# glmanhtu/vit-ed

Hardware: AMD Instinct MI355X
Metric: patch-pairs/sec fwd+bwd, div2k_erosion7_4bin_patch8_64 ViT-ED (higher is better)
Workload: dtype bf16

## Files before the change

### profiles/row_probe.py

```python
#!/usr/bin/env python3
import argparse
import os
import sys

import torch

sys.path.insert(0, os.path.dirname(os.path.dirname(os.path.abspath(__file__))))
import vited_amd as v

ops, L = v.ops, v._lib


def main():
    ap = argparse.ArgumentParser()
    ap.add_argument('--reps', type=int, default=10)
    ap.add_argument('--rows', type=int, nargs='*', default=[65536, 66560])
    a = ap.parse_args()
    dev = torch.device('cuda:0')
    g = torch.Generator(device='cpu').manual_seed(0)

    def rnd(*shape, scale=1.0):
        return (torch.randn(*shape, generator=g) * scale).to(dev)

    def timed(fn):
        for _ in range(3):
            fn()
        torch.cuda.synchronize()
        e0, e1 = torch.cuda.Event(enable_timing=True), torch.cuda.Event(enable_timing=True)
        e0.record()
        for _ in range(a.reps):
            fn()
        e1.record()
        torch.cuda.synchronize()
        return e0.elapsed_time(e1) / a.reps * 1e3

    N = 384
    print(f'{"shape":28s} {"two kernels":>12s} {"fused":>9s}   GB/s (fused, algorithmic)')
    for M in a.rows:
        gamma, beta, bias = 1.0 + rnd(N, scale=0.1), rnd(N, scale=0.1), rnd(N, scale=0.1)
        res = rnd(M, N)
        mean, rstd = rnd(M, scale=0.1), 1.0 + rnd(M, scale=0.1).abs()
        for K in (384, 768, 1152, 1536):
            x_lp, w = rnd(M, K).bfloat16(), rnd(N, K, scale=K ** -0.5).bfloat16()

            def fwd_two():
                y = ops.gemm(x_lp, w, epilogue=L.EPI_RESIDUAL, bias=bias, residual=res)
                return ops.layernorm_fwd(y, gamma, beta, 1e-6, torch.bfloat16)

            def fwd_fused():
                return ops.linear_residual_layernorm_fwd(x_lp, w, bias, res, gamma, beta, 1e-6)

            def bwd_two():
                dh = ops.gemm(x_lp, w)
                return ops.layernorm_bwd(dh, res, gamma, mean, rstd, dx_in=res, want_lp=True)

            def bwd_fused():
                return ops.linear_layernorm_bwd(x_lp, w, res, gamma, mean, rstd, dx_in=res, want_lp=True)

            t2, t1 = timed(fwd_two), timed(fwd_fused)
            byt = M * K * 2 + N * K * 2 + M * N * (4 + 4 + 2)
            print(f'fwd M={M} K={K:5d}          {t2:10.1f}us {t1:8.1f}us   {byt / t1 / 1e3:7.0f}   {2.0 * M * N * K / t1 / 1e6:6.0f} TF/s')
            t2, t1 = timed(bwd_two), timed(bwd_fused)
            byt = M * K * 2 + N * K * 2 + M * N * (4 + 4 + 4 + 2)
            print(f'bwd M={M} K={K:5d}          {t2:10.1f}us {t1:8.1f}us   {byt / t1 / 1e3:7.0f}   {2.0 * M * N * K / t1 / 1e6:6.0f} TF/s')


if __name__ == '__main__':
    main()
```

### vit-ed_amd/csrc/gemm_row.hip

```cpp
#include <mutex>
#include <type_traits>

#include "gemm_kernels.h"
#include "gemm_lds.h"

#define ROW_N 384
#define ROW_LD 388

enum { ROW_MODE_FWD = 0, ROW_MODE_BWD = 1 };

struct RowArgs {
    const bf16* A; int64_t lda;
    int seg_k; int64_t seg_stride;
    const bf16* W; int64_t ldw;
    int64_t M; int K;
    const float* bias; const float* residual; int64_t ldr;
    float* y; int64_t ldy;
    const float* gamma; const float* beta; float eps;
    bf16* h; int64_t ldh; float* mean; float* rstd;
    const float* x; int64_t ldx; const float* mean_in; const float* rstd_in;
    const float* dx_in; int64_t ldxi; float* dx; int64_t lddx; bf16* dx_lp; int64_t ldlp;
    float* partial;
};

template <int MT> struct RowCfg {
    static_assert(MT == 6 || MT == 8 || MT == 9 || MT == 10, "tile heights: 96, 128, 144 or 160 rows");
    static constexpr int BM = 16 * MT;
    static constexpr int A_BYTES = BM * 128;
    static constexpr int W_BYTES = ROW_N * 128;
    static constexpr int W_BASE = 3 * A_BYTES;
    static constexpr int LDS_BYTES = 3 * A_BYTES + 2 * W_BYTES;
    static constexpr int P0 = (MT + 1) / 2;
    static constexpr int A_PIECES = 2 * MT;
    static constexpr int A_J = (A_PIECES + 3) / 4;
    static constexpr int PASS_SUB = MT == 8 ? 4 : MT == 10 ? 5 : 3;
    static constexpr int PASS_ROWS = 16 * PASS_SUB;
    static constexpr int NPASS = MT / PASS_SUB;
    static constexpr int ROWS_PER_HALF = PASS_ROWS / 16;
    static constexpr bool EPI_ALL_ROWS = MT <= 9;
    static_assert(MT % PASS_SUB == 0, "passes cover the tile");
    static_assert(LDS_BYTES <= 160 * 1024, "LDS");
    static_assert(LDS_BYTES >= PASS_ROWS * ROW_LD * 4, "epilogue scratch must fit the staging buffers");
    static_assert(LDS_BYTES >= 16 * 2 * ROW_N * 4, "column-partial combine must fit the staging buffers");
};

__device__ __forceinline__ float row_half_sum(float v) { return half_wave_sum(v); }

#define ROW_STORE(ptr, val) __builtin_nontemporal_store(val, ptr)
#define ROW_STORE_LP(ptr, val) (*(ptr) = (val))
#define ROW_LOAD(ptr) __builtin_nontemporal_load(ptr)

struct RowFwdIn { f32x4 res[3]; };
struct RowBwdIn { f32x4 x[3], din[3]; float mu, rs; };

template <int MODE, int MT>
__global__ void __launch_bounds__(512)
gemm_row_kernel(const RowArgs a) {
    extern __shared__ __attribute__((aligned(16))) char smem[];
    using R = RowCfg<MT>;
    const int lane = threadIdx.x & 63;
    const int wave = __builtin_amdgcn_readfirstlane(threadIdx.x >> 6);
    const int64_t m0 = (int64_t)blockIdx.x * R::BM;

    f32x4 acc[MT][3];
#pragma unroll
    for (int i = 0; i < MT; ++i)
#pragma unroll
        for (int j = 0; j < 3; ++j) acc[i][j] = f32x4{0.f, 0.f, 0.f, 0.f};

    const int grp = wave >> 2, u = wave & 3;
    const int nt = a.K / 64;
    const int r8 = lane >> 3, c8 = lane & 7;
    const int cs_even = (c8 ^ (r8 >> 1)) * 8, cs_odd = (c8 ^ (r8 >> 1) ^ 4) * 8;
    const int cs_u = (u & 1) ? cs_odd : cs_even;
    const int a_per = (R::A_PIECES - u + 3) / 4;
    const bf16* pa[R::A_J];
#pragma unroll
    for (int j = 0; j < R::A_J; ++j) {
        int64_t ar = m0 + 8 * (4 * j + u) + r8;
#ifdef ROW_DBG_A_RESIDENT
        ar -= m0;
#endif
        ar = ar < a.M ? ar : a.M - 1;
        pa[j] = a.A + ar * a.lda + cs_u;
    }
    const bf16* pw = a.W + (int64_t)(8 * u + r8) * a.ldw + cs_u;
    auto issue_a = [&](int t) {
#ifdef ROW_DBG_NO_DMA
        return;
#endif
        if (t >= nt) return;
        char* dst = smem + (t % 3) * R::A_BYTES;
        const int k0 = t * 64;
        const int seg = k0 / a.seg_k;
        const int64_t ka = (int64_t)seg * a.seg_stride + (k0 - seg * a.seg_k);
#pragma unroll
        for (int j = 0; j < R::A_J; ++j)
            if (4 * j + 3 < R::A_PIECES || j < a_per) glds16_asm(pa[j] + ka, dst + (4 * j + u) * 1024);
    };
    auto issue_w = [&](int t, int part) {
#ifdef ROW_DBG_NO_DMA
        return;
#endif
        if (t >= nt) return;
        char* dst = smem + R::W_BASE + (t & 1) * R::W_BYTES + (16 * part + u) * 1024;
        const int64_t off = (int64_t)(128 * part) * a.ldw + t * 64;
#pragma unroll
        for (int j = 0; j < 4; ++j) glds16_asm(pw + off + (int64_t)(32 * j) * a.ldw, dst + 4 * j * 1024);
    };
    const int fr = lane & 15, fq = lane >> 4;
    const int loff0 = fr * 128 + ((fq ^ ((fr >> 1) & 7)) << 4), loff1 = fr * 128 + (((4 + fq) ^ ((fr >> 1) & 7)) << 4);
    bf16x8 fa[R::P0][2] = {}, fb[3][2] = {};
    auto read_b = [&](int t) {
#ifdef ROW_DBG_NO_READS
        return;
#endif
        const char* wb = smem + R::W_BASE + (t & 1) * R::W_BYTES + wave * 48 * 128;
#pragma unroll
        for (int j = 0; j < 3; ++j) {
            fb[j][0] = *(const bf16x8*)(wb + j * 2048 + loff0);
            fb[j][1] = *(const bf16x8*)(wb + j * 2048 + loff1);
        }
    };
    auto read_a = [&](int t, auto i0_tag, auto n_tag) {
        constexpr int I0 = decltype(i0_tag)::value, NR = decltype(n_tag)::value;
#ifdef ROW_DBG_NO_READS
        return;
#endif
        const char* ab = smem + (t % 3) * R::A_BYTES + I0 * 2048;
#pragma unroll
        for (int i = 0; i < NR; ++i) {
            fa[i][0] = *(const bf16x8*)(ab + i * 2048 + loff0);
            fa[i][1] = *(const bf16x8*)(ab + i * 2048 + loff1);
        }
    };
    auto mfmas = [&](auto i0_tag, auto n_tag) {
        constexpr int I0 = decltype(i0_tag)::value, NR = decltype(n_tag)::value;
        __builtin_amdgcn_s_setprio(1);
#pragma unroll
        for (int kk = 0; kk < 2; ++kk)
#pragma unroll
            for (int i = 0; i < NR; ++i)
#pragma unroll
                for (int j = 0; j < 3; ++j)
#ifdef ROW_DBG_NO_MFMA
                    asm volatile("" ::"v"(fb[j][kk]), "v"(fa[i][kk]));
#else
                    acc[I0 + i][j] = __builtin_amdgcn_mfma_f32_16x16x32_bf16(fb[j][kk], fa[i][kk], acc[I0 + i][j], 0, 0, 0);
#endif
        __builtin_amdgcn_s_setprio(0);
    };
    auto barrier = [&]() {
        __builtin_amdgcn_s_barrier();
        asm volatile("" ::: "memory");
    };
    auto certify_barrier = [&](bool younger) {
        __builtin_amdgcn_sched_barrier(0);
        if (!younger) asm volatile("s_waitcnt vmcnt(0)\n\ts_barrier" ::: "memory");
        else if (grp == 0 && a_per == 5) asm volatile("s_waitcnt vmcnt(5)\n\ts_barrier" ::: "memory");
        else if (grp == 0 && a_per == 3) asm volatile("s_waitcnt vmcnt(3)\n\ts_barrier" ::: "memory");
        else asm volatile("s_waitcnt vmcnt(4)\n\ts_barrier" ::: "memory");
        __builtin_amdgcn_sched_barrier(0);
    };
    auto landed = [&]() {
#ifndef ROW_DBG_LATE_LGKM
        __builtin_amdgcn_s_waitcnt(0xc07f);
#endif
    };
    using I0 = std::integral_constant<int, 0>;
    using IP0 = std::integral_constant<int, R::P0>;
    using IP1 = std::integral_constant<int, MT - R::P0>;
    if (grp == 0) {
        issue_a(0);
        issue_w(0, 1);
        issue_a(1);
        certify_barrier(nt > 1);
        for (int t = 0; t < nt; ++t) {
            read_b(t);
            read_a(t, I0{}, IP0{});
            issue_w(t + 1, 1);
            landed();
            barrier();
            mfmas(I0{}, IP0{});
            barrier();
            read_a(t, IP0{}, IP1{});
            issue_a(t + 2);
            landed();
            barrier();
            mfmas(IP0{}, IP1{});
            certify_barrier(t + 2 < nt);
        }
        barrier();
    } else {
        issue_w(0, 0);
        issue_w(0, 2);
        issue_w(1, 0);
        certify_barrier(nt > 1);
        barrier();
        for (int t = 0; t < nt; ++t) {
            read_b(t);
            read_a(t, I0{}, IP0{});
            issue_w(t + 1, 2);
            landed();
            barrier();
            mfmas(I0{}, IP0{});
            barrier();
            read_a(t, IP0{}, IP1{});
            issue_w(t + 2, 0);
            landed();
            certify_barrier(t + 2 < nt);
            mfmas(IP0{}, IP1{});
            barrier();
        }
    }
#ifdef ROW_DBG_NO_EPI
#pragma unroll
    for (int i = 0; i < MT; ++i)
#pragma unroll
        for (int j = 0; j < 3; ++j) asm volatile("" ::"v"(acc[i][j]));
    return;
#endif

    float* sc = (float*)smem;
    const int hl = lane & 31;
    const int hw = wave * 2 + (lane >> 5);
    const float inv_d = 1.0f / ROW_N;
    f32x4 gm[3], bt[3], bs[3];
#pragma unroll
    for (int j = 0; j < 3; ++j) {
        const int c = (j * 32 + hl) * 4;
        gm[j] = a.gamma ? *(const f32x4*)(a.gamma + c) : f32x4{1.f, 1.f, 1.f, 1.f};
        bt[j] = (MODE == ROW_MODE_FWD && a.beta) ? *(const f32x4*)(a.beta + c) : f32x4{0.f, 0.f, 0.f, 0.f};
        bs[j] = (MODE == ROW_MODE_FWD && a.bias) ? *(const f32x4*)(a.bias + c) : f32x4{0.f, 0.f, 0.f, 0.f};
    }
    f32x4 dg[3], db[3];
#pragma unroll
    for (int j = 0; j < 3; ++j) {
        dg[j] = f32x4{0.f, 0.f, 0.f, 0.f};
        db[j] = f32x4{0.f, 0.f, 0.f, 0.f};
    }
    auto load_fwd = [&](RowFwdIn& in, int64_t m) {
        const bool ok = m < a.M;
#pragma unroll
        for (int j = 0; j < 3; ++j)
            in.res[j] = ok ? ROW_LOAD((const f32x4*)(a.residual + m * a.ldr + (j * 32 + hl) * 4)) : f32x4{0.f, 0.f, 0.f, 0.f};
    };
    auto load_bwd = [&](RowBwdIn& in, int64_t m) {
        const bool ok = m < a.M;
#pragma unroll
        for (int j = 0; j < 3; ++j) {
            const int c = (j * 32 + hl) * 4;
            in.x[j] = ok ? ROW_LOAD((const f32x4*)(a.x + m * a.ldx + c)) : f32x4{0.f, 0.f, 0.f, 0.f};
            in.din[j] = (ok && a.dx_in) ? ROW_LOAD((const f32x4*)(a.dx_in + m * a.ldxi + c)) : f32x4{0.f, 0.f, 0.f, 0.f};
        }
        in.mu = ok ? a.mean_in[m] : 0.f;
        in.rs = ok ? a.rstd_in[m] : 0.f;
    };
    auto row_fwd = [&](const RowFwdIn& in, int r, int64_t m) {
        if (m >= a.M) return;
        f32x4 v[3];
        float s = 0.f;
#pragma unroll
        for (int j = 0; j < 3; ++j) {
            const int c = (j * 32 + hl) * 4;
            v[j] = *(const f32x4*)(sc + r * ROW_LD + c);
#pragma unroll
            for (int e = 0; e < 4; ++e) {
                v[j][e] += bs[j][e];
                v[j][e] += in.res[j][e];
            }
            ROW_STORE((f32x4*)(a.y + m * a.ldy + c), v[j]);
            s += (v[j][0] + v[j][1]) + (v[j][2] + v[j][3]);
        }
        if (!a.h) return;
        const float mu = row_half_sum(s) * inv_d;
        float q = 0.f;
#pragma unroll
        for (int j = 0; j < 3; ++j)
#pragma unroll
            for (int e = 0; e < 4; ++e) {
                const float d = v[j][e] - mu;
                q = fmaf(d, d, q);
            }
        const float rs = rsqrtf(row_half_sum(q) * inv_d + a.eps);
#pragma unroll
        for (int j = 0; j < 3; ++j) {
            const int c = (j * 32 + hl) * 4;
            bf16x4 o;
#pragma unroll
            for (int e = 0; e < 4; ++e) o[e] = (bf16)((v[j][e] - mu) * rs * gm[j][e] + bt[j][e]);
            ROW_STORE_LP((bf16x4*)(a.h + m * a.ldh + c), o);
        }
        if (hl == 0) {
            a.mean[m] = mu;
            a.rstd[m] = rs;
        }
    };
    auto row_bwd = [&](const RowBwdIn& in, int r, int64_t m) {
        if (m >= a.M) return;
        f32x4 xh[3], gg[3];
        float s1 = 0.f, s2 = 0.f;
#pragma unroll
        for (int j = 0; j < 3; ++j) {
            const int c = (j * 32 + hl) * 4;
            const f32x4 d = *(const f32x4*)(sc + r * ROW_LD + c);
#pragma unroll
            for (int e = 0; e < 4; ++e) {
                xh[j][e] = (in.x[j][e] - in.mu) * in.rs;
                gg[j][e] = d[e] * gm[j][e];
                s1 += gg[j][e];
                s2 = fmaf(gg[j][e], xh[j][e], s2);
                dg[j][e] = fmaf(d[e], xh[j][e], dg[j][e]);
                db[j][e] += d[e];
            }
        }
        const float c1 = row_half_sum(s1) * inv_d, c2 = row_half_sum(s2) * inv_d;
#pragma unroll
        for (int j = 0; j < 3; ++j) {
            const int c = (j * 32 + hl) * 4;
            f32x4 v;
#pragma unroll
            for (int e = 0; e < 4; ++e) v[e] = in.rs * (gg[j][e] - c1 - xh[j][e] * c2) + in.din[j][e];
            ROW_STORE((f32x4*)(a.dx + m * a.lddx + c), v);
            if (a.dx_lp) ROW_STORE_LP((bf16x4*)(a.dx_lp + m * a.ldlp + c), (bf16x4{(bf16)v[0], (bf16)v[1], (bf16)v[2], (bf16)v[3]}));
        }
    };

#pragma unroll
    for (int p = 0; p < R::NPASS; ++p) {
        const int64_t mp = m0 + p * R::PASS_ROWS;
        constexpr int AHEAD = R::EPI_ALL_ROWS ? R::ROWS_PER_HALF : 1;
        RowFwdIn fin[AHEAD + (R::EPI_ALL_ROWS ? 0 : 1)];
        RowBwdIn bin[AHEAD + (R::EPI_ALL_ROWS ? 0 : 1)];
#pragma unroll
        for (int k = 0; k < AHEAD; ++k) {
            if (MODE == ROW_MODE_FWD) load_fwd(fin[k], mp + hw + 16 * k);
            else load_bwd(bin[k], mp + hw + 16 * k);
        }
        __syncthreads();
#pragma unroll
        for (int ii = 0; ii < R::PASS_SUB; ++ii) {
            const int i = R::PASS_SUB * p + ii;
#pragma unroll
            for (int j = 0; j < 3; ++j) *(f32x4*)(sc + (ii * 16 + fr) * ROW_LD + wave * 48 + j * 16 + fq * 4) = acc[i][j];
        }
        __syncthreads();
#pragma unroll
        for (int k = 0; k < R::ROWS_PER_HALF; ++k) {
            const int r = hw + 16 * k;
            if constexpr (R::EPI_ALL_ROWS) {
                if (MODE == ROW_MODE_FWD) row_fwd(fin[k], r, mp + r);
                else row_bwd(bin[k], r, mp + r);
            } else {
                const bool more = k + 1 < R::ROWS_PER_HALF;
                if (MODE == ROW_MODE_FWD) {
                    if (more) load_fwd(fin[(k + 1) & 1], mp + r + 16);
                    row_fwd(fin[k & 1], r, mp + r);
                } else {
                    if (more) load_bwd(bin[(k + 1) & 1], mp + r + 16);
                    row_bwd(bin[k & 1], r, mp + r);
                }
            }
        }
    }

    if (MODE == ROW_MODE_BWD) {
        __syncthreads();
        float* my = sc + hw * 2 * ROW_N;
#pragma unroll
        for (int j = 0; j < 3; ++j) {
            const int c = (j * 32 + hl) * 4;
            *(f32x4*)(my + c) = dg[j];
            *(f32x4*)(my + ROW_N + c) = db[j];
        }
        __syncthreads();
        float* out = a.partial + (int64_t)blockIdx.x * 2 * ROW_N;
        for (int c = threadIdx.x; c < 2 * ROW_N; c += 512) {
            float s = 0.f;
#pragma unroll
            for (int w = 0; w < 16; ++w) s += sc[w * 2 * ROW_N + c];
            out[c] = s;
        }
    }
}

static inline int row_mt(int64_t M) {
    static const int heights[] = {10, 9, 8, 6};
    int best = 8;
    int64_t cost = -1;
    for (int mt : heights) {
        const int64_t c = ceil_div64(ceil_div64(M, 16 * mt), 256) * mt;
        if (cost < 0 || c < cost) {
            cost = c;
            best = mt;
        }
    }
    return best;
}

static inline int64_t row_tiles(int64_t M) { return ceil_div64(M, 16 * row_mt(M)); }

static bool row_shape_ok(int64_t M, int64_t N, int64_t K) { return N == ROW_N && K >= 64 && K % 64 == 0 && K <= (1 << 20) && M >= 1 && M < ((int64_t)1 << 31); }

extern "C" int vited_linear_layernorm_supported(int64_t M, int64_t N, int64_t K) { return row_shape_ok(M, N, K) ? 1 : 0; }

template <int MODE, int MT>
static int row_launch_mt(const RowArgs& a, unsigned tiles, hipStream_t s) {
    auto kernel = gemm_row_kernel<MODE, MT>;
    static std::once_flag once;
    static hipError_t status = hipSuccess;
    std::call_once(once, [&] { status = hipFuncSetAttribute((const void*)kernel, hipFuncAttributeMaxDynamicSharedMemorySize, RowCfg<MT>::LDS_BYTES); });
    if (status != hipSuccess) return VITED_ERR_LAUNCH;
    hipLaunchKernelGGL(kernel, dim3(tiles), dim3(512), RowCfg<MT>::LDS_BYTES, s, a);
    return vited_check_launch();
}

template <int MODE>
static int row_launch(const RowArgs& a, hipStream_t s) {
    const unsigned tiles = (unsigned)row_tiles(a.M);
    switch (row_mt(a.M)) {
        case 6: return row_launch_mt<MODE, 6>(a, tiles, s);
        case 9: return row_launch_mt<MODE, 9>(a, tiles, s);
        case 10: return row_launch_mt<MODE, 10>(a, tiles, s);
        default: return row_launch_mt<MODE, 8>(a, tiles, s);
    }
}

static inline bool al16(const void* p) { return ((uintptr_t)p & 15) == 0; }

extern "C" int vited_linear_residual_layernorm_fwd(const void* a, int64_t lda, const void* w, int64_t ldw, const float* bias,
                                                   const float* residual, int64_t ldr, float* y, int64_t ldy, const float* gamma,
                                                   const float* beta, float eps, void* h, int64_t ldh, float* mean, float* rstd,
                                                   int64_t M, int64_t N, int64_t K, void* stream) {
    if (!a || !w || !residual || !y || M <= 0 || N <= 0 || K <= 0 || lda < K || ldw < K || ldr < N || ldy < N) return VITED_ERR_BAD_ARG;
    if (h && (!gamma || !beta || !mean || !rstd || ldh < N)) return VITED_ERR_BAD_ARG;
    if (!row_shape_ok(M, N, K)) return VITED_ERR_UNSUPPORTED;
    if ((lda & 7) || (ldw & 7) || (ldr & 3) || (ldy & 3) || (h && (ldh & 3))) return VITED_ERR_UNSUPPORTED;
    if (!al16(a) || !al16(w) || !al16(residual) || !al16(y) || !al16(bias) || !al16(gamma) || !al16(beta) || ((uintptr_t)h & 7))
        return VITED_ERR_BAD_ARG;
    RowArgs r = {};
    r.A = (const bf16*)a; r.lda = lda; r.seg_k = (int)K; r.seg_stride = 0; r.W = (const bf16*)w; r.ldw = ldw; r.M = M; r.K = (int)K;
    r.bias = bias; r.residual = residual; r.ldr = ldr; r.y = y; r.ldy = ldy;
    r.gamma = gamma; r.beta = beta; r.eps = eps; r.h = (bf16*)h; r.ldh = ldh; r.mean = mean; r.rstd = rstd;
    return row_launch<ROW_MODE_FWD>(r, (hipStream_t)stream);
}

int ln_bwd_finish(const float* partial, int nparts, int dim, float* dgamma, float* dbeta, int accumulate, hipStream_t s);

extern "C" int64_t vited_linear_layernorm_bwd_partial_rows(int64_t M) { return M >= 1 ? row_tiles(M) : 0; }

extern "C" int64_t vited_linear_layernorm_bwd_workspace_bytes(int64_t M, int64_t N) {
    return N == ROW_N && M >= 1 ? row_tiles(M) * 2 * ROW_N * (int64_t)sizeof(float) : 0;
}

static int linear_layernorm_bwd_impl(const void* dy, int64_t lddy, int64_t seg_k, int64_t seg_stride, const void* wt, int64_t ldwt,
                                    const float* x, int64_t ldx, const float* gamma, const float* mean, const float* rstd,
                                    const float* dx_in, int64_t dx_in_ld, float* dx_out, int64_t dx_out_ld, void* dx_lp, int64_t dx_lp_ld,
                                    float* dgamma, float* dbeta, int accumulate, int64_t M, int64_t N, int64_t K, float* workspace,
                                    int64_t workspace_bytes, void* stream) {
    if (!dy || !wt || !x || !gamma || !mean || !rstd || !dx_out || M <= 0 || N <= 0 || K <= 0) return VITED_ERR_BAD_ARG;
    if ((dgamma == nullptr) != (dbeta == nullptr)) return VITED_ERR_BAD_ARG;
    if (seg_k <= 0 || K % seg_k || lddy < seg_k || ldwt < K || ldx < N || dx_out_ld < N || (dx_in && dx_in_ld < N) || (dx_lp && dx_lp_ld < N))
        return VITED_ERR_BAD_ARG;
    if (!row_shape_ok(M, N, K) || seg_k % 64 || (seg_stride & 7)) return VITED_ERR_UNSUPPORTED;
    if ((lddy & 7) || (ldwt & 7) || (ldx & 3) || (dx_out_ld & 3) || (dx_in && (dx_in_ld & 3)) || (dx_lp && (dx_lp_ld & 3))) return VITED_ERR_UNSUPPORTED;
    if (!al16(dy) || !al16(wt) || !al16(x) || !al16(gamma) || !al16(dx_in) || !al16(dx_out) || ((uintptr_t)dx_lp & 7)) return VITED_ERR_BAD_ARG;
    if (!workspace || workspace_bytes < vited_linear_layernorm_bwd_workspace_bytes(M, N)) return VITED_ERR_WORKSPACE;
    RowArgs r = {};
    r.A = (const bf16*)dy; r.lda = lddy; r.seg_k = (int)seg_k; r.seg_stride = seg_stride; r.W = (const bf16*)wt; r.ldw = ldwt; r.M = M; r.K = (int)K;
    r.gamma = gamma; r.x = x; r.ldx = ldx; r.mean_in = mean; r.rstd_in = rstd;
    r.dx_in = dx_in; r.ldxi = dx_in_ld; r.dx = dx_out; r.lddx = dx_out_ld; r.dx_lp = (bf16*)dx_lp; r.ldlp = dx_lp_ld;
    r.partial = workspace;
    const int rc = row_launch<ROW_MODE_BWD>(r, (hipStream_t)stream);
    if (rc != VITED_OK || !dgamma) return rc;
    return ln_bwd_finish(workspace, (int)row_tiles(M), ROW_N, dgamma, dbeta, accumulate, (hipStream_t)stream);
}

extern "C" int vited_linear_layernorm_bwd(const void* dy, int64_t lddy, const void* wt, int64_t ldwt, const float* x, int64_t ldx,
                                          const float* gamma, const float* mean, const float* rstd, const float* dx_in,
                                          int64_t dx_in_ld, float* dx_out, int64_t dx_out_ld, void* dx_lp, int64_t dx_lp_ld,
                                          float* dgamma, float* dbeta, int accumulate, int64_t M, int64_t N, int64_t K,
                                          float* workspace, int64_t workspace_bytes, void* stream) {
    return linear_layernorm_bwd_impl(dy, lddy, K, 0, wt, ldwt, x, ldx, gamma, mean, rstd, dx_in, dx_in_ld, dx_out, dx_out_ld, dx_lp, dx_lp_ld,
                                     dgamma, dbeta, accumulate, M, N, K, workspace, workspace_bytes, stream);
}

extern "C" int vited_linear_layernorm_bwd_segmented(const void* dy, int64_t lddy, int64_t seg_k, int64_t seg_stride, int64_t segments,
                                                    const void* wt, int64_t ldwt, const float* x, int64_t ldx, const float* gamma,
                                                    const float* mean, const float* rstd, const float* dx_in, int64_t dx_in_ld,
                                                    float* dx_out, int64_t dx_out_ld, void* dx_lp, int64_t dx_lp_ld, float* dgamma,
                                                    float* dbeta, int accumulate, int64_t M, int64_t N, float* workspace,
                                                    int64_t workspace_bytes, void* stream) {
    if (segments <= 0) return VITED_ERR_BAD_ARG;
    return linear_layernorm_bwd_impl(dy, lddy, seg_k, seg_stride, wt, ldwt, x, ldx, gamma, mean, rstd, dx_in, dx_in_ld, dx_out, dx_out_ld, dx_lp,
                                     dx_lp_ld, dgamma, dbeta, accumulate, M, N, segments * seg_k, workspace, workspace_bytes, stream);
}
```

Before: 43060.

## Prefetch next epilogue pass inputs and add persistent-kernel probe variants

Across epilogue passes of the fused linear+layernorm kernel, the residual or activation rows for the next pass are now loaded into registers before the current pass's row work, so global-load latency overlaps with computation. Separately, compile-time probe options add a persistent tile loop and a dummy epilogue interleaved into the main loop, plus a fused-only timing flag in the probe script. The default build gets only the prefetch, which raises register pressure in exchange for the latency hiding.

```diff
diff --git a/profiles/row_probe.py b/profiles/row_probe.py
--- a/profiles/row_probe.py
+++ b/profiles/row_probe.py
@@ -15,6 +15,7 @@
     ap = argparse.ArgumentParser()
     ap.add_argument('--reps', type=int, default=10)
     ap.add_argument('--rows', type=int, nargs='*', default=[65536, 66560])
+    ap.add_argument('--fused-only', action='store_true', help='time only the fused kernel (variant builds: VITED_LIB=...)')
     a = ap.parse_args()
     dev = torch.device('cuda:0')
     g = torch.Generator(device='cpu').manual_seed(0)
@@ -57,10 +58,10 @@
             def bwd_fused():
                 return ops.linear_layernorm_bwd(x_lp, w, res, gamma, mean, rstd, dx_in=res, want_lp=True)
 
-            t2, t1 = timed(fwd_two), timed(fwd_fused)
+            t2, t1 = (0.0 if a.fused_only else timed(fwd_two)), timed(fwd_fused)
             byt = M * K * 2 + N * K * 2 + M * N * (4 + 4 + 2)
             print(f'fwd M={M} K={K:5d}          {t2:10.1f}us {t1:8.1f}us   {byt / t1 / 1e3:7.0f}   {2.0 * M * N * K / t1 / 1e6:6.0f} TF/s')
-            t2, t1 = timed(bwd_two), timed(bwd_fused)
+            t2, t1 = (0.0 if a.fused_only else timed(bwd_two)), timed(bwd_fused)
             byt = M * K * 2 + N * K * 2 + M * N * (4 + 4 + 4 + 2)
             print(f'bwd M={M} K={K:5d}          {t2:10.1f}us {t1:8.1f}us   {byt / t1 / 1e3:7.0f}   {2.0 * M * N * K / t1 / 1e6:6.0f} TF/s')
 
diff --git a/vit-ed_amd/csrc/gemm_row.hip b/vit-ed_amd/csrc/gemm_row.hip
--- a/vit-ed_amd/csrc/gemm_row.hip
+++ b/vit-ed_amd/csrc/gemm_row.hip
@@ -38,6 +38,8 @@
     static constexpr int NPASS = MT / PASS_SUB;
     static constexpr int ROWS_PER_HALF = PASS_ROWS / 16;
     static constexpr bool EPI_ALL_ROWS = MT <= 9;
+    static constexpr int PF_FWD = EPI_ALL_ROWS ? ROWS_PER_HALF : 0;
+    static constexpr int PF_BWD = EPI_ALL_ROWS ? 1 : 0;
     static_assert(MT % PASS_SUB == 0, "passes cover the tile");
     static_assert(LDS_BYTES <= 160 * 1024, "LDS");
     static_assert(LDS_BYTES >= PASS_ROWS * ROW_LD * 4, "epilogue scratch must fit the staging buffers");
@@ -60,7 +62,74 @@
     using R = RowCfg<MT>;
     const int lane = threadIdx.x & 63;
     const int wave = __builtin_amdgcn_readfirstlane(threadIdx.x >> 6);
-    const int64_t m0 = (int64_t)blockIdx.x * R::BM;
+#if defined(ROW_PROBE_DUMMY_EPI) && !defined(ROW_PROBE_PERSIST)
+#error "ROW_PROBE_DUMMY_EPI needs ROW_PROBE_PERSIST"
+#endif
+#ifdef ROW_PROBE_PERSIST
+    const int64_t n_tiles = (a.M + R::BM - 1) / R::BM;
+    const int64_t tile_end = (int64_t)(blockIdx.x + 1) * n_tiles / gridDim.x;
+#ifdef ROW_PROBE_DUMMY_EPI
+    int64_t dm0 = -1;
+    int dnext = 0;
+    f32x4 dq[3] = {}, dr[3] = {};
+    float dmu = 0.f, drs = 0.f;
+    auto dummy_item = [&]() {
+        if (dm0 < 0 || dnext > MT) return;
+        const int hl = lane & 31, hw = wave * 2 + (lane >> 5);
+        if (dnext > 0) {
+            const int64_t m = dm0 + 16 * (dnext - 1) + hw;
+            if (m < a.M) {
+#pragma unroll
+                for (int j = 0; j < 3; ++j) {
+                    const int c = (j * 32 + hl) * 4;
+                    f32x4 v;
+#pragma unroll
+                    for (int e = 0; e < 4; ++e) v[e] = MODE == ROW_MODE_FWD ? dq[j][e] + 1.f : (dq[j][e] - dmu) * drs + dr[j][e];
+                    const bf16x4 o = {(bf16)v[0], (bf16)v[1], (bf16)v[2], (bf16)v[3]};
+                    if (MODE == ROW_MODE_FWD) {
+                        ROW_STORE((f32x4*)(a.y + m * a.ldy + c), v);
+                        if (a.h) ROW_STORE_LP((bf16x4*)(a.h + m * a.ldh + c), o);
+                    } else {
+                        ROW_STORE((f32x4*)(a.dx + m * a.lddx + c), v);
+                        if (a.dx_lp) ROW_STORE_LP((bf16x4*)(a.dx_lp + m * a.ldlp + c), o);
+                    }
+                }
+                if (MODE == ROW_MODE_FWD && a.h && hl == 0) {
+                    a.mean[m] = dq[0][0];
+                    a.rstd[m] = dq[0][1];
+                }
+            }
+        }
+        if (dnext < MT) {
+            const int64_t m = dm0 + 16 * dnext + hw;
+            const bool ok = m < a.M;
+#pragma unroll
+            for (int j = 0; j < 3; ++j) {
+                const int c = (j * 32 + hl) * 4;
+                if (MODE == ROW_MODE_FWD) {
+                    dq[j] = ok ? ROW_LOAD((const f32x4*)(a.residual + m * a.ldr + c)) : f32x4{0.f, 0.f, 0.f, 0.f};
+                } else {
+                    dq[j] = ok ? ROW_LOAD((const f32x4*)(a.x + m * a.ldx + c)) : f32x4{0.f, 0.f, 0.f, 0.f};
+                    dr[j] = (ok && a.dx_in) ? ROW_LOAD((const f32x4*)(a.dx_in + m * a.ldxi + c)) : f32x4{0.f, 0.f, 0.f, 0.f};
+                }
+            }
+            if (MODE == ROW_MODE_BWD) {
+                dmu = ok ? a.mean_in[m] : 0.f;
+                drs = ok ? a.rstd_in[m] : 0.f;
+            }
+        }
+        ++dnext;
+    };
+#define ROW_PROBE_SLOT() dummy_item()
+#endif
+    for (int64_t tile = (int64_t)blockIdx.x * n_tiles / gridDim.x; tile < tile_end; ++tile) {
+#else
+    const int64_t tile = blockIdx.x;
+#endif
+#ifndef ROW_PROBE_SLOT
+#define ROW_PROBE_SLOT()
+#endif
+    const int64_t m0 = tile * R::BM;
 
     f32x4 acc[MT][3];
 #pragma unroll
@@ -179,12 +248,14 @@
             read_b(t);
             read_a(t, I0{}, IP0{});
             issue_w(t + 1, 1);
+            ROW_PROBE_SLOT();
             landed();
             barrier();
             mfmas(I0{}, IP0{});
             barrier();
             read_a(t, IP0{}, IP1{});
             issue_a(t + 2);
+            ROW_PROBE_SLOT();
             landed();
             barrier();
             mfmas(IP0{}, IP1{});
@@ -201,25 +272,36 @@
             read_b(t);
             read_a(t, I0{}, IP0{});
             issue_w(t + 1, 2);
+            ROW_PROBE_SLOT();
             landed();
             barrier();
             mfmas(I0{}, IP0{});
             barrier();
             read_a(t, IP0{}, IP1{});
             issue_w(t + 2, 0);
+            ROW_PROBE_SLOT();
             landed();
             certify_barrier(t + 2 < nt);
             mfmas(IP0{}, IP1{});
             barrier();
         }
     }
-#ifdef ROW_DBG_NO_EPI
+#if defined(ROW_DBG_NO_EPI) || defined(ROW_PROBE_DUMMY_EPI)
 #pragma unroll
     for (int i = 0; i < MT; ++i)
 #pragma unroll
         for (int j = 0; j < 3; ++j) asm volatile("" ::"v"(acc[i][j]));
+#ifdef ROW_PROBE_DUMMY_EPI
+    while (dm0 >= 0 && dnext <= MT) dummy_item();
+    dm0 = m0;
+    dnext = 0;
+    }
+    while (dnext <= MT) dummy_item();
+#elif defined(ROW_PROBE_PERSIST)
+    }
+#endif
     return;
-#endif
+#else
 
     float* sc = (float*)smem;
     const int hl = lane & 31;
@@ -326,16 +408,24 @@
         }
     };
 
+    constexpr int AHEAD = R::EPI_ALL_ROWS ? R::ROWS_PER_HALF : 1;
+    constexpr int PF = MODE == ROW_MODE_FWD ? R::PF_FWD : R::PF_BWD;
+    RowFwdIn fpre[PF > 0 ? PF : 1];
+    RowBwdIn bpre[PF > 0 ? PF : 1];
 #pragma unroll
     for (int p = 0; p < R::NPASS; ++p) {
         const int64_t mp = m0 + p * R::PASS_ROWS;
-        constexpr int AHEAD = R::EPI_ALL_ROWS ? R::ROWS_PER_HALF : 1;
         RowFwdIn fin[AHEAD + (R::EPI_ALL_ROWS ? 0 : 1)];
         RowBwdIn bin[AHEAD + (R::EPI_ALL_ROWS ? 0 : 1)];
 #pragma unroll
         for (int k = 0; k < AHEAD; ++k) {
-            if (MODE == ROW_MODE_FWD) load_fwd(fin[k], mp + hw + 16 * k);
-            else load_bwd(bin[k], mp + hw + 16 * k);
+            if (p > 0 && k < PF) {
+                if (MODE == ROW_MODE_FWD) fin[k] = fpre[k];
+                else bin[k] = bpre[k];
+            } else {
+                if (MODE == ROW_MODE_FWD) load_fwd(fin[k], mp + hw + 16 * k);
+                else load_bwd(bin[k], mp + hw + 16 * k);
+            }
         }
         __syncthreads();
 #pragma unroll
@@ -345,6 +435,13 @@
             for (int j = 0; j < 3; ++j) *(f32x4*)(sc + (ii * 16 + fr) * ROW_LD + wave * 48 + j * 16 + fq * 4) = acc[i][j];
         }
         __syncthreads();
+        if (p + 1 < R::NPASS) {
+#pragma unroll
+            for (int k = 0; k < PF; ++k) {
+                if (MODE == ROW_MODE_FWD) load_fwd(fpre[k], mp + R::PASS_ROWS + hw + 16 * k);
+                else load_bwd(bpre[k], mp + R::PASS_ROWS + hw + 16 * k);
+            }
+        }
 #pragma unroll
         for (int k = 0; k < R::ROWS_PER_HALF; ++k) {
             const int r = hw + 16 * k;
@@ -374,7 +471,7 @@
             *(f32x4*)(my + ROW_N + c) = db[j];
         }
         __syncthreads();
-        float* out = a.partial + (int64_t)blockIdx.x * 2 * ROW_N;
+        float* out = a.partial + tile * 2 * ROW_N;
         for (int c = threadIdx.x; c < 2 * ROW_N; c += 512) {
             float s = 0.f;
 #pragma unroll
@@ -382,6 +479,11 @@
             out[c] = s;
         }
     }
+#ifdef ROW_PROBE_PERSIST
+    __syncthreads();
+    }
+#endif
+#endif
 }
 
 static inline int row_mt(int64_t M) {
@@ -411,6 +513,9 @@
     static hipError_t status = hipSuccess;
     std::call_once(once, [&] { status = hipFuncSetAttribute((const void*)kernel, hipFuncAttributeMaxDynamicSharedMemorySize, RowCfg<MT>::LDS_BYTES); });
     if (status != hipSuccess) return VITED_ERR_LAUNCH;
+#ifdef ROW_PROBE_PERSIST
+    tiles = tiles < 256 ? tiles : 256;
+#endif
     hipLaunchKernelGGL(kernel, dim3(tiles), dim3(512), RowCfg<MT>::LDS_BYTES, s, a);
     return vited_check_launch();
 }
```

Measured after the change: 43150 (median of 6 runs). Within noise of the previous version (+0.2%).
